# joaotavora/raytracing-one-weekend

Measured on AMD Instinct MI355X. Metric: Msamples/sec (W×H×spp) on cover scene; achieved HBM GB/s vs peak, higher is better.
Workload: dtype f64

## Files before the change

### include/rtow.h

```cpp
#ifndef RTOW_H
#define RTOW_H

#include <stdint.h>

#ifdef __cplusplus
extern "C" {
#endif

#define RTOW_ABI_VERSION 9

#define RTOW_OK 0
#define RTOW_EINVAL (-1)
#define RTOW_ENODEV (-2)
#define RTOW_EHIP (-3)
#define RTOW_ENOSCENE (-4)
#define RTOW_EEMPTY (-5)
#define RTOW_ENOMEM (-6)

#define RTOW_MAT_LAMBERTIAN 0
#define RTOW_MAT_METAL 1
#define RTOW_MAT_DIELECTRIC 2

#define RTOW_PRIM_SPHERE 0
#define RTOW_PRIM_MOVING_SPHERE 1
// ... 101 lines not shown
  int32_t bvh_image_bytes;
  int32_t grid_image_bytes;
  double bvh_build_ms;
  double grid_build_ms;
  double upload_ms;
  int32_t bvh4_nodes;
  int32_t bvh4_image_bytes;
  int32_t ref_tree_nodes;
  int32_t bvh4_node_bytes;
  double ref_tree_stupid_volume;
  double ref_tree_build_ms;
} rtow_build_info_t;
int rtow_build_info(rtow_ctx *ctx, rtow_build_info_t *out);

int rtow_local_rows(const rtow_config_t *cfg);
int rtow_local_row_list(const rtow_config_t *cfg, int32_t *rows_out, int32_t capacity);

int rtow_render_device(rtow_ctx *ctx, const rtow_config_t *cfg, void *d_rgb_sums,
                       void *hip_stream, rtow_stats_t *stats);

int rtow_render_device_rgb8(rtow_ctx *ctx, const rtow_config_t *cfg, void *d_rgb8, void *hip_stream,
                            rtow_stats_t *stats);

int rtow_tonemap_device(rtow_ctx *ctx, const void *d_rgb_sums, int64_t n_values, int32_t spp_effective,
                        void *d_rgb8, void *hip_stream);

int rtow_profile_collect(rtow_ctx *ctx, double *kernel_ms_sum, int32_t *launches);

int rtow_debug_counters(rtow_ctx *ctx, unsigned long long *out48);

int rtow_debug_schedule(rtow_ctx *ctx, const rtow_config_t *cfg, uint32_t *out_pairs, int32_t capacity_pairs);

int rtow_debug_last_spec(rtow_ctx *ctx, uint32_t *out_spec);

int rtow_debug_tile_order(const rtow_scene_t *scene, const rtow_config_t *cfg, uint32_t *table_out, unsigned char *empty_out,
                          int32_t capacity, int32_t *n_empty, int32_t *tile_w_log2, int32_t *tile_h_log2);

int rtow_debug_image(rtow_ctx *ctx, int32_t which, void *out, int64_t capacity, int64_t *size_out);

typedef struct rtow_ray_t {
  double origin[3];
  double time;
  double direction[3];
  double tmax;
} rtow_ray_t;

typedef struct rtow_hit_t {
  double t;
  double point[3];
  double normal[3];
  int32_t prim;
  int32_t kind;
  int32_t material;
  int32_t front_face;
} rtow_hit_t;

int rtow_intersect_device(rtow_ctx *ctx, int32_t precision, int32_t kernel, const void *d_rays, int64_t n_rays,
                          void *d_hits, void *hip_stream, rtow_stats_t *stats);
int rtow_intersect(rtow_ctx *ctx, int32_t precision, int32_t kernel, const rtow_ray_t *rays, int64_t n_rays,
                   rtow_hit_t *hits, rtow_stats_t *stats);

int rtow_occluded_device(rtow_ctx *ctx, int32_t precision, int32_t kernel, const void *d_rays, int64_t n_rays,
                         void *d_occluded , void *hip_stream, rtow_stats_t *stats);
int rtow_occluded(rtow_ctx *ctx, int32_t precision, int32_t kernel, const rtow_ray_t *rays, int64_t n_rays,
                  uint8_t *occluded, rtow_stats_t *stats);

// ... 126 lines not shown
```

### raytracing-one-weekend_amd/csrc/rtow_capi.cpp

```cpp

#include <hip/hip_runtime.h>

#include <cmath>
#include <cstdarg>
#include <cstdio>
#include <cstdlib>
#include <algorithm>
#include <chrono>
#include <cstring>
#include <string>
#include <vector>

#include "../../include/rtow.h"
#include "rtow_bvh.h"
#include "rtow_bvh4.h"
#include "rtow_device.h"
#include "rtow_grid.h"
#include "rtow_reftree.h"

namespace {

thread_local std::string g_err;

int fail(int code, const char *fmt, ...) {
// ... 241 lines not shown
struct Knobs {
  int bvh_leaf = 0;
  double bvh_ct = -1.0;
  bool no_leaf_order = false;
  double grid_cpp = 1.0;
  double grid_large = 4.0;
  int grid_max_tris = 8192;
  unsigned long long partials_cap = 8ull << 30;
  int bvh_block = 0;
  int blocks_per_cu = 0;
  bool no_tiles = false;
  int sky_eighths = 1;
  bool stamps = false;
  bool bvh4_no_aux = false;
  bool no_bvh4 = false;
  int fetch_votes = 0;
  int leaf_votes = 0;
  int walk_cap = -1, walk_max_open = 0;
  bool bvh4_sm = false;
  int sm4_votes[3] = {8, 16, 16};
  int bvh4_stack_k = 0;
  int sched_chunk = 10;
  int sched_chunk_mesh = 16;
  int ploc_radius = -1;
  int device_tree = 2;
  bool stream_scalar = false;
  bool no_spec = false;
  bool no_flat = false;
  bool tile_order = true;
  int empty_levels = 3;
  int tail_bound = 0;
  int radiance_blocks = 0;
  int guides_blocks = 0;
  void read() {
    auto geti = [](const char *n, int d) { const char *e = std::getenv(n); return e ? std::atoi(e) : d; };
    auto getd = [](const char *n, double d) { const char *e = std::getenv(n); return e ? std::atof(e) : d; };
    bvh_leaf = geti("RTOW_BVH_LEAF", 0);
    bvh_ct = getd("RTOW_BVH_CT", -1.0);
    no_leaf_order = std::getenv("RTOW_NO_LEAF_ORDER") != nullptr;
    grid_cpp = getd("RTOW_GRID_CPP", 1.0);
    grid_large = getd("RTOW_GRID_LARGE", 4.0);
    grid_max_tris = geti("RTOW_GRID_MAX_TRIS", 8192);
    if (const char *e = std::getenv("RTOW_PARTIALS_MAX_MB")) partials_cap = (unsigned long long)std::atoll(e) << 20;
    bvh_block = geti("RTOW_BVH_BLOCK", 0);
    if (bvh_block != 256 && bvh_block != 512 && bvh_block != 1024) bvh_block = 0;
    blocks_per_cu = geti("RTOW_BLOCKS_PER_CU", 0);
    if (blocks_per_cu < 1 || blocks_per_cu > 16) blocks_per_cu = 0;
    no_tiles = std::getenv("RTOW_NO_TILES") != nullptr;
    sky_eighths = std::min(std::max(geti("RTOW_SKY_EIGHTHS", 1), 0), 8);
    stamps = std::getenv("RTOW_STAMPS") != nullptr;
    no_bvh4 = std::getenv("RTOW_NO_BVH4") != nullptr;
    bvh4_no_aux = std::getenv("RTOW_BVH4_NO_AUX") != nullptr;
    fetch_votes = std::min(std::max(geti("RTOW_FETCH_VOTES", 0), 0), 64);
    leaf_votes = std::min(std::max(geti("RTOW_LEAF_VOTES", 0), 0), 64);
    bvh4_sm = std::getenv("RTOW_BVH4_SM") != nullptr;
    if (const char *e = std::getenv("RTOW_WALK_CAP")) {
      int a = 0, b = 0;
      if (std::sscanf(e, "%d,%d", &a, &b) == 2 && a > 0 && b > 0) {
        walk_cap = a;
        walk_max_open = std::min(b, 64);
      } else {
        walk_cap = 0;
      }
    }
    if (const char *e = std::getenv("RTOW_SM4_VOTES")) {
      int a = 0, b = 0, d = 0;
      if (std::sscanf(e, "%d,%d,%d", &a, &b, &d) == 3) {
        sm4_votes[0] = std::min(std::max(a, 1), 64);
        sm4_votes[1] = std::min(std::max(b, 1), 64);
        sm4_votes[2] = std::min(std::max(d, 1), 64);
      }
    }
    bvh4_stack_k = std::min(std::max(geti("RTOW_BVH4_STACK_K", 0), 0), 64);
    sched_chunk = std::min(std::max(geti("RTOW_SCHED_CHUNK", 10), 0), 4096);
    sched_chunk_mesh = std::min(std::max(geti("RTOW_SCHED_CHUNK_MESH", 16), 0), 4096);
    tail_bound = std::max(geti("RTOW_TAIL_BOUND", 0), 0);
    radiance_blocks = std::max(geti("RTOW_RADIANCE_BLOCKS", 0), 0);
    guides_blocks = std::max(geti("RTOW_GUIDES_BLOCKS", 0), 0);
    tile_order = geti("RTOW_TILE_ORDER", 1) != 0;
    empty_levels = std::min(std::max(geti("RTOW_EMPTY_LEVELS", 3), 1), 16);
    no_spec = std::getenv("RTOW_NO_SPEC") != nullptr;
    no_flat = std::getenv("RTOW_NO_FLAT") != nullptr;
    stream_scalar = std::getenv("RTOW_STREAM_SCALAR") != nullptr;
    if (const char *e = std::getenv("RTOW_PLOC_RADIUS")) ploc_radius = std::min(std::max(std::atoi(e), 0), 64);
    if (const char *e = std::getenv("RTOW_DEVICE_TREE"))
      device_tree = std::strcmp(e, "radix") == 0 ? 0 : (std::strcmp(e, "ploc") == 0 ? 1 : 2);
    if (ploc_radius >= 0 && !std::getenv("RTOW_DEVICE_TREE")) device_tree = ploc_radius == 0 ? 0 : 1;
  }
};

constexpr unsigned kNeedBvh = 1u, kNeedGrid = 2u, kNeedF32 = 4u, kNeedBvh4 = 8u, kNeedAll = 15u;

struct rtow_ctx {
  int device = 0;
  Knobs knobs;
  int num_cus = 0;
  bool have_scene = false;
  rtow::DevScene ds{};
  rtow::DevCamera cam{};
  int n_prims = 0;
  DevBuf sph, sph_r, mov, tri, tri16, prim_mat, mats, blob, cam_dev, gblob;
  DevBuf blob4;
  bool have_bvh4 = false;
  bool have_tri16 = false;
  int bvh4_depth = 0;
  DevBuf blob32, gblob32, cam32_dev;
  rtow::DevScene ds32{};
  uint32_t gblob_bytes = 0;
  uint32_t grid_fat_stride = 0;
  int32_t grid_ny = 0;
  GridWalkConsts grid_walk{};
// ... 1122 lines not shown
  LaunchShape shape;
  if ((rc = launch_shape(c, kernel, f32, shape))) return rc;
  rtow::DevScene &scene = shape.scene;
  const int block = shape.block;
  const unsigned lds_bytes = shape.lds_bytes;
  const int stack_bound = shape.stack_bound;
  const bool image_kernel = shape.image_kernel;

  if (stats) {
    std::memset(stats, 0, sizeof *stats);
    stats->local_rows = rows;
    stats->kernel_used = kernel;
  }
  if (npix == 0) return RTOW_OK;
  if (spt == 0) {
    if (!accumulate) HIPCHK(hipMemsetAsync(d_rgb_sums, 0, (size_t)npix * 3 * sizeof(double), st));
    if (stats) HIPCHK(hipStreamSynchronize(st));
    return RTOW_OK;
  }

  int &occ = c->occ[strict ? 0 : (f32 ? 2 : 1)][kernel - 1];
  if (kernel == RTOW_KERNEL_BVH4) occ = 0;
  if (occ <= 0) {
    occ = strict ? rtow::trace_occupancy_strict(kernel, block, lds_bytes)
          : f32  ? rtow::trace_occupancy_f32(kernel, block, lds_bytes)
                 : rtow::trace_occupancy_fast(kernel, block, lds_bytes);
    if (occ <= 0) return fail(RTOW_EHIP, "occupancy query failed (kernel %d, %u B of LDS)", kernel, lds_bytes);
    if (occ > 8) occ = 8;
    if (c->knobs.blocks_per_cu) occ = c->knobs.blocks_per_cu;
  }
  long long grid = (long long)c->num_cus * occ;
  const long long need_blocks = (long long)((n_items + block - 1) / block);
  if (grid > need_blocks) grid = need_blocks;
  if (grid < 1) grid = 1;
  const unsigned long long n_lanes = (unsigned long long)grid * block;

  const size_t depth_slots = (size_t)(cfg->max_child_rays > 0 ? cfg->max_child_rays : 1);
  if ((rc = c->partials.ensure((size_t)n_items * 3 * sizeof(double))) ||
      (rc = c->stack.ensure(strict ? depth_slots * (size_t)n_lanes * sizeof(uint32_t) : 4)) ||
      (rc = c->counters.ensure(48 * sizeof(unsigned long long))))
    return rc;
  if (kernel == RTOW_KERNEL_BVH4) {
    const int extra = std::max(stack_bound - (int)scene.b4_stack_k, 0);
    if ((rc = c->spill.ensure(std::max<size_t>((size_t)extra * (size_t)n_lanes * sizeof(uint32_t), 16)))) return rc;
  }

#ifdef RTOW_TAILSTAT
  if (kernel == RTOW_KERNEL_BVH4) return fail(RTOW_EINVAL, "RTOW_TAILSTAT builds do not run the BVH4 kernel");
  if ((rc = c->spill.ensure(std::max<size_t>((size_t)n_lanes, 16)))) return rc;
#endif
  rtow::TraceParams P;
  std::memset(&P, 0, sizeof P);
  P.sc = scene;
  P.cam = (const rtow::DevCamera *)c->cam_dev.p;
  P.cam32 = (const float *)c->cam32_dev.p;
  P.W = cfg->image_width;
  P.H = cfg->image_height;
  P.spt = spt;
  P.nstreams = streams_now;
  P.stream_first = plan.first + lvl_first;
  P.sample_base = (uint32_t)(plan.base + (long long)lvl_first * spt);
  P.spt_last = spt_last;
  {
    const unsigned long long b = 64ull * (4096ull + 8ull * (unsigned long long)(cfg->max_child_rays + 2) *
                                                        (unsigned long long)(std::max(spt, spt_last) + 1));
    P.tail_bound = c->knobs.tail_bound > 0 ? (uint32_t)c->knobs.tail_bound : (uint32_t)std::min<unsigned long long>(b, 0xfffffff0ull);
  }
  P.dropped = (unsigned long long *)c->dropped.p;
  P.inv_wm1 = 1.0 / (double)(cfg->image_width - 1);
  P.inv_hm1 = 1.0 / (double)(cfg->image_height - 1);
  P.max_child_rays = cfg->max_child_rays;
  P.rank = cfg->rank;
  P.nranks = cfg->nranks;
  P.tile_rows = cfg->tile_rows;
  P.local_rows = rows;
  P.seed_lo = (uint32_t)cfg->seed;
  P.seed_hi = (uint32_t)(cfg->seed >> 32);
  P.n_items = (uint32_t)n_items;
  P.n_lanes = (uint32_t)n_lanes;
  P.npix_local = (uint32_t)npix;
  P.div_npix = make_fastdiv((uint32_t)npix);
  P.div_w = make_fastdiv((uint32_t)cfg->image_width);
// ... 26 lines not shown
    }
    P.tile_table = (const uint32_t *)c->tile_table.p;
    P.n_items_first = P.n_items - c->tile_empty * 64u * (uint32_t)streams_now;
    P.empty_batch = 64u * (uint32_t)c->knobs.empty_levels;
  }
  P.partials = (double *)c->partials.p;
  P.stack = (uint32_t *)c->stack.p;
  P.spill = (uint32_t *)c->spill.p;
  P.spec = rtow::kSpecGeneric;
  if (kernel == RTOW_KERNEL_GRID && lds_bytes > 0 && !f32 && !c->knobs.no_spec && scene.n_tri == 0) {
    if (scene.n_mov == 0 && c->grid_fat_stride == 48u) P.spec = rtow::kSpecStaticSpheres;
    if (scene.n_mov > 0 && c->grid_fat_stride == 80u) P.spec = rtow::kSpecMovingSpheres;
    if (P.spec != rtow::kSpecGeneric && c->grid_ny == 1 && !c->knobs.no_flat) P.spec |= rtow::kSpecFlatY;
  }
  P.walk = c->grid_walk;
  P.b4_trips = c->knobs.bvh4_sm ? 0u : 1u;
  {
    const bool b4 = kernel == RTOW_KERNEL_BVH4;
    const bool b4_nodes_resident = b4 && scene.b4_lds_limit >= scene.b4_off_tri;
    int cap = c->knobs.walk_cap, open = c->knobs.walk_max_open;
    if (cap < 0) {
      cap = b4 ? 4 : 3;
      open = b4 ? (b4_nodes_resident ? 24 : 32) : 16;
    }
    if (cap > 0 && !b4) cap = std::max(cap, 3);
    P.walk_cap = cap > 0 ? (uint32_t)cap : 0xffffffffu;
    P.walk_max_open = (uint32_t)open;
    P.leaf_votes = (uint32_t)(c->knobs.leaf_votes > 0 ? c->knobs.leaf_votes : (b4 ? 28 : 16));
  }
  P.fetch_votes = (uint32_t)(c->knobs.fetch_votes > 0 ? c->knobs.fetch_votes : (kernel == RTOW_KERNEL_BVH4 ? 2 : 4));
  P.sm4_restart = (uint32_t)c->knobs.sm4_votes[0];
  P.sm4_scatter = (uint32_t)c->knobs.sm4_votes[1];
  P.sm4_leaf = (uint32_t)c->knobs.sm4_votes[2];
  P.counters = (unsigned long long *)c->counters.p;
  P.t_origin = P.counters + 16;

  if (st != nullptr) HIPCHK(hipStreamWaitEvent(st, c->upload_ev, 0));
  if (stats) HIPCHK(hipEventRecord(c->call_ev[0], st));
  if (!c->counters_init.p) {
    std::vector<unsigned long long> init(48, 0ull);
    init[5] = init[16] = ~0ull;
    if ((rc = c->counters_init.ensure(48 * sizeof(unsigned long long)))) return rc;
    HIPCHK(hipMemcpy(c->counters_init.p, init.data(), 48 * sizeof(unsigned long long), hipMemcpyHostToDevice));
  }
  HIPCHK(hipMemcpyAsync(c->counters.p, c->counters_init.p, 48 * sizeof(unsigned long long), hipMemcpyDeviceToDevice, st));
  const int slot = c->ev_count < kEventRing ? c->ev_count : -1;
  if (slot >= 0) HIPCHK(hipEventRecord(c->ev[slot][0], st));
  int launch_kernel = kernel;
  if (image_kernel && lds_bytes > 0 && c->knobs.stamps) launch_kernel = kernel + 16;
  int lrc = strict ? rtow::launch_trace_strict(P, launch_kernel, (int)grid, block, lds_bytes, st)
            : f32  ? rtow::launch_trace_f32(P, launch_kernel, (int)grid, block, lds_bytes, st)
                   : rtow::launch_trace_fast(P, launch_kernel, (int)grid, block, lds_bytes, st);
#ifdef RTOW_TAILSTAT
  if (const char *path = std::getenv("RTOW_TAILSTAT_OUT")) {
    HIPCHK(hipStreamSynchronize(st));
    std::vector<unsigned long long> ts((size_t)n_lanes / 64 * 8);
    HIPCHK(hipMemcpy(ts.data(), c->spill.p, ts.size() * 8, hipMemcpyDeviceToHost));
    if (FILE *f = std::fopen(path, "wb")) {
      std::fwrite(ts.data(), 8, ts.size(), f);
      std::fclose(f);
    }
  }
#endif
  if (lrc != 0) return fail(RTOW_EHIP, "trace kernel launch failed: %s", hipGetErrorString((hipError_t)lrc));
  c->last_spec = (int64_t)P.spec;
  if (slot >= 0) {
    HIPCHK(hipEventRecord(c->ev[slot][1], st));
    c->ev_count++;
  }
  rtow::ReduceParams R;
  R.partials = P.partials;
  R.out = (double *)d_rgb_sums;
  R.npix3 = (uint32_t)(npix * 3);
  R.nstreams = streams_now;
  R.accumulate = accumulate;
  R.W = (uint32_t)cfg->image_width;
  R.tile_w_log2 = tw;
  R.tile_h_log2 = th;
  R.tiles_per_row = P.div_tpr_n;
  R.rgb8 = nullptr;
  R.spp = 0.0;
  if (c->fuse_rgb8 && lvl_first == 0 && lvl_count == plan.count && !accumulate) {
    R.rgb8 = c->fuse_rgb8;
    R.spp = c->fuse_spp;
    c->fuse_used = true;
  }
  lrc = rtow::launch_reduce(R, st);
  if (lrc != 0) return fail(RTOW_EHIP, "reduce kernel launch failed: %s", hipGetErrorString((hipError_t)lrc));

// ... 553 lines not shown
        frame.half = c->ds.b4_half;
        frame.lds_limit = c->ds.b4_lds_limit;
        bytes = (int64_t)sizeof frame;
      }
      break;
    default: return fail(RTOW_EINVAL, "unknown image %d", which);
  }
  *size_out = bytes;
  if (!out) return RTOW_OK;
  if (capacity < bytes) return fail(RTOW_EINVAL, "buffer too small (%lld < %lld)", (long long)capacity, (long long)bytes);
  if (which == 5) {
    if (bytes) std::memcpy(out, &frame, sizeof frame);
    return RTOW_OK;
  }
  HIPCHK(hipSetDevice(c->device));
  HIPCHK(hipDeviceSynchronize());
  if (bytes) HIPCHK(hipMemcpy(out, src, (size_t)bytes, hipMemcpyDeviceToHost));
  return RTOW_OK;
}

int rtow_debug_counters(rtow_ctx *c, unsigned long long *out48) {
  if (!c || !out48) return fail(RTOW_EINVAL, "NULL argument");
  if (!c->counters.p) return fail(RTOW_ENOSCENE, "no launch yet");
  HIPCHK(hipSetDevice(c->device));
  HIPCHK(hipDeviceSynchronize());
  HIPCHK(hipMemcpy(out48, c->counters.p, 48 * sizeof(unsigned long long), hipMemcpyDeviceToHost));
  return RTOW_OK;
}

int rtow_debug_last_spec(rtow_ctx *c, uint32_t *out_spec) {
  if (!c || !out_spec) return fail(RTOW_EINVAL, "NULL argument");
  if (c->last_spec < 0) return fail(RTOW_ENOSCENE, "no launch yet");
  *out_spec = (uint32_t)c->last_spec;
  return RTOW_OK;
}

int rtow_tonemap_device(rtow_ctx *c, const void *d_rgb_sums, int64_t n_values, int32_t spp_effective,
                        void *d_rgb8, void *hip_stream) {
  if (!c) return fail(RTOW_EINVAL, "ctx is NULL");
  if (!d_rgb_sums || !d_rgb8) return fail(RTOW_EINVAL, "NULL device pointer");
  if (n_values < 0 || n_values > 0xffffffffLL) return fail(RTOW_EINVAL, "n_values out of range");
  if (spp_effective <= 0) return fail(RTOW_EINVAL, "spp_effective must be positive");
  HIPCHK(hipSetDevice(c->device));
  int lrc = rtow::launch_tonemap((const double *)d_rgb_sums, (unsigned char *)d_rgb8, (uint32_t)n_values,
                                 (double)spp_effective, hip_stream);
  if (lrc != 0) return fail(RTOW_EHIP, "tonemap launch failed: %s", hipGetErrorString((hipError_t)lrc));
  return RTOW_OK;
}

int rtow_profile_collect(rtow_ctx *c, double *kernel_ms_sum, int32_t *launches) {
  if (!c) return fail(RTOW_EINVAL, "ctx is NULL");
  HIPCHK(hipSetDevice(c->device));
  double sum = 0.0;
  for (int i = 0; i < c->ev_count; ++i) {
    HIPCHK(hipEventSynchronize(c->ev[i][1]));
    float ms = 0.f;
    HIPCHK(hipEventElapsedTime(&ms, c->ev[i][0], c->ev[i][1]));
    sum += ms;
  }
  if (kernel_ms_sum) *kernel_ms_sum = sum;
  if (launches) *launches = c->ev_count;
  const bool waited = c->ev_count > 0;
  c->ev_count = 0;
  return waited ? check_dropped(c, false) : RTOW_OK;
}

// ... 515 lines not shown
```

### raytracing-one-weekend_amd/csrc/rtow_device.h

```cpp
#pragma once
#include <stdint.h>

#include "rtow_walk_consts.h"

namespace rtow {

struct DevMaterial {
  double att[3];
  double fuzz;
  double ir;
  int32_t kind;
  int32_t pad_;
};

struct DevCamera {
  double origin[3], u[3], v[3];
  double horizontal[3], vertical[3], llc[3];
  double lens_radius, t0, t1;
};

struct DevScene {
  const double *sph;
  const double *sph_r;
  const double *mov;
// ... 51 lines not shown
};
struct alignas(32) FetchHead {
  uint32_t n_items;
  uint32_t n_items_first;
  uint32_t empty_batch;
  int32_t W;
  double *partials;
  unsigned long long *counters;
};
static_assert(sizeof(FetchDecode) == 128 && sizeof(FetchHead) == 32, "aligned runs: one or two wide scalar loads each");

struct TraceParams : FetchDecode, FetchHead {
  DevScene sc;
  const DevCamera *cam;
  const float *cam32;
  int32_t H;
  int32_t stream_first;
  uint32_t tail_bound;
  double inv_wm1, inv_hm1;
  int32_t max_child_rays;
  int32_t local_rows;
  uint32_t seed_lo, seed_hi;
  uint32_t n_lanes;
  FastDiv div_npix, div_w;
  uint32_t n_tile_rows;
  uint32_t *stack;
  uint32_t *spill;
  uint32_t spec;
  uint32_t b4_trips;
  uint32_t fetch_votes;
  uint32_t leaf_votes;
  uint32_t walk_cap, walk_max_open;
  uint32_t sm4_restart, sm4_scatter, sm4_leaf;
  unsigned long long *dropped;
  unsigned long long *t_origin;
  GridWalkConsts walk;
};

constexpr uint32_t kSpecGeneric = 0u, kSpecStaticSpheres = 1u, kSpecMovingSpheres = 2u;
constexpr uint32_t kSpecFlatY = 4u;

struct ReduceParams {
  const double *partials;
  double *out;
  uint32_t npix3;
  int32_t nstreams;
  int32_t accumulate;
  uint32_t W, tile_w_log2, tile_h_log2, tiles_per_row;
  unsigned char *rgb8;
  double spp;
};

int launch_trace_strict(const TraceParams &p, int kernel, int grid, int block, unsigned lds_bytes,
                        void *stream);
int launch_trace_fast(const TraceParams &p, int kernel, int grid, int block, unsigned lds_bytes,
                      void *stream);
int launch_trace_f32(const TraceParams &p, int kernel, int grid, int block, unsigned lds_bytes,
                     void *stream);
int trace_occupancy_strict(int kernel, int block, unsigned lds_bytes);
int trace_occupancy_fast(int kernel, int block, unsigned lds_bytes);
int trace_occupancy_f32(int kernel, int block, unsigned lds_bytes);
int launch_reduce(const ReduceParams &p, void *stream);
int launch_tonemap(const double *sums, unsigned char *rgb8, uint32_t n, double spp, void *stream);
int launch_place_rows(const void *gathered, void *image, uint32_t n_ranks, uint32_t max_rows, uint32_t row_bytes,
                      uint32_t height, uint32_t tile_rows, void *stream);

}
```

### raytracing-one-weekend_amd/csrc/rtow_trace_body.h

```cpp

#include <hip/hip_runtime.h>
#include <stdint.h>
#include <type_traits>

#include "rtow_device.h"

#ifndef RTOW_SUFFIX
#error "define RTOW_SUFFIX"
#endif
#define RTOW_CAT2(a, b) a##b
#define RTOW_CAT(a, b) RTOW_CAT2(a, b)

namespace rtow {
namespace {
#include "rtow_trace_math.h"
#include "rtow_trace_rng.h"
#include "rtow_trace_hit.h"
#include "rtow_trace_stamps.h"
#include "rtow_trace_bvh.h"
#include "rtow_trace_grid.h"
#include "rtow_trace_bvh4.h"
#ifndef RTOW_FAST_MATH
#include "rtow_trace_reftree.h"
#endif
// ... 202 lines not shown
  const unsigned lane = lane_id();
  [[maybe_unused]] const uint32_t lane_g = blockIdx.x * blockDim.x + threadIdx.x;

  Image<LDS> im;
  [[maybe_unused]] Bvh4Reader<LDS> im4;
  stage_scene<KERNEL, LDS>(sc, im, im4);

  bool done = false;
  bool need_sample = true;
  bool pending_hit = false;
  int s_left = 0;
  uint32_t item = 0xffffffffu;
  uint32_t j = 0;
  uint32_t gi = 0;
  V3d acc = {0.0, 0.0, 0.0};
  V3 ro = {0, 0, 0}, rd = {0, 0, 1};
  real rtime = 0;
  int depth = 0;
  [[maybe_unused]] int nb = 0;
#ifdef RTOW_FAST_MATH
  V3 throughput = {1, 1, 1};
#endif
  Rng g = {0, 0, 0};
  uint32_t nseg = 0, nnode = 0, nprim = 0;
  [[maybe_unused]] float t_resume = 0.0f;
  [[maybe_unused]] uint32_t w_cur = 0x1fffffu, w_sa = 0u;
  Closest best;
  best.t = 0;
  best.prim = -1;
  bool helping = false;
  bool holding = false;
  uint32_t partners = 0u;
  int n_out = 0;
  uint32_t tail_left = P.tail_bound;
  asm volatile("" : "+v"(tail_left));
  ItemPool pool;
  const uint32_t n_waves = (gridDim.x * blockDim.x) >> 6;
#ifdef RTOW_TAILSTAT
  unsigned long long ts_start = __builtin_amdgcn_s_memrealtime(), ts_empty = 0ull;
  uint32_t ts_trips = 0u, ts_trips_after = 0u, ts_live = 0u, ts_left = 0u, ts_pool = 0u;
#endif
  Stamps<STAMPS> stamps;
  stamps.start();
  unsigned long long t_empty = 0ull;
  unsigned long long trips_after_empty = 0ull;
  if constexpr (STAMPS) {
    if (lane == 0) atomicMin(P.t_origin, (unsigned long long)__builtin_amdgcn_s_memrealtime());
  }

  for (;;) {
    bool need_item = false;
    if (!done && need_sample && s_left <= 0) {
      if (helping) {
        helping = false;
        holding = true;
        done = true;
      } else if (n_out == 0) {
        need_item = true;
      }
    }
    unsigned long long need_mask = __ballot(need_item);
    if (need_mask != 0ull && (uint32_t)__popcll(need_mask) < P.fetch_votes && __ballot(!done && !need_item) != 0ull) {
      need_mask = 0ull;
      need_item = false;
    }
    if (need_mask != 0ull) {
      const RTOW_CONST TraceParams *kp = (const RTOW_CONST TraceParams *)__builtin_amdgcn_kernarg_segment_ptr();
      asm volatile("" : "+s"(kp));
      const FetchHead fh = load_fetch_head(kp);
      if (need_item && item != 0xffffffffu) {
        double *dst = fh.partials + (size_t)item * 3;
        dst[0] = acc.x;
        dst[1] = acc.y;
        dst[2] = acc.z;
        item = 0xffffffffu;
      }
      const unsigned long long mine = take_items(pool, need_mask, lane, n_waves, fh);
      if (need_item) {
        if (mine >= (unsigned long long)fh.n_items) {
          done = true;
#ifdef RTOW_TAILSTAT
          if (ts_empty == 0ull) ts_empty = 1ull;
#endif
          if constexpr (STAMPS) {
            if (t_empty == 0ull) t_empty = __builtin_amdgcn_s_memrealtime();
          }
        } else {
          const ItemPos ip = decode_item(kp, fh, (uint32_t)mine);
          item = ip.item;
          j = ip.j;
          gi = ip.gi;
          g.pixel = gi * (uint32_t)fh.W + j;
          g.sample = ip.sample0;
          s_left = ip.count;
          acc = {0.0, 0.0, 0.0};
        }
      }
    }
#ifdef RTOW_TAILSTAT
    {
      const bool first = __ballot(ts_empty == 1ull) != 0ull && __ballot(ts_empty > 1ull) == 0ull;
      if (first) {
        const unsigned long long now = __builtin_amdgcn_s_memrealtime();
        ts_live = (uint32_t)__popcll(__ballot(!done));
        uint32_t sl = (!done && s_left > 0) ? (uint32_t)s_left : 0u;
        for (int off = 32; off >= 1; off >>= 1) sl += __shfl_xor(sl, off);
        ts_left = sl;
        ts_pool = pool.end - pool.next;
        ts_empty = now < 2ull ? 2ull : now;
      } else if (__ballot(ts_empty > 1ull) != 0ull) {
        ts_empty = (unsigned long long)__shfl((long long)ts_empty, __ffsll((long long)__ballot(ts_empty > 1ull)) - 1);
      }
      ++ts_trips;
      if (__ballot(ts_empty > 1ull) != 0ull) ++ts_trips_after;
    }
#endif
    if (__ballot(done) != 0ull) {
#ifdef RTOW_DONATE_R2
      const bool ready = !done && need_sample && s_left <= 0 && n_out > 0;
      if (__ballot(ready) != 0ull) {
        const uint32_t h = partners & 63u;
        const uint32_t src = ready ? h : lane;
        const uint32_t partner_holds = lane_read(src, (uint32_t)holding);
        const bool take = ready && partner_holds != 0u;
        const V3d c = {lane_read(src, acc.x), lane_read(src, acc.y), lane_read(src, acc.z)};
        const uint32_t ow = holding ? partners : lane;
        const bool o_take = lane_read(ow, (uint32_t)take) != 0u;
        const uint32_t o_h = lane_read(ow, h);
        if (take) {
          acc = acc + c;
          partners >>= 6;
          --n_out;
        }
        if (holding && o_take && o_h == lane) holding = false;
      }
      const bool can_give = !done && !helping && s_left >= 2 && n_out < 5;
#else
      unsigned long long rm = __ballot(!done && need_sample && s_left <= 0 && n_out > 0);
      while (rm != 0ull) {
        const int o = __ffsll((long long)rm) - 1;
        rm &= rm - 1ull;
        const uint32_t want_sample = (uint32_t)__builtin_amdgcn_readlane((int)g.sample, o);
        const uint32_t want_pixel = (uint32_t)__builtin_amdgcn_readlane((int)g.pixel, o);
        const unsigned long long held =
            __ballot(holding && partners == (uint32_t)o && g.sample == want_sample + 1u && g.pixel == want_pixel);
        if (held != 0ull) {
          const int h = __ffsll((long long)held) - 1;
          const V3d c = {wave_bcast_f64(acc.x, h), wave_bcast_f64(acc.y, h), wave_bcast_f64(acc.z, h)};
          if ((int)lane == o) {
            acc = acc + c;
            ++g.sample;
            --n_out;
          }
          if ((int)lane == h) holding = false;
          if (__builtin_amdgcn_readlane(n_out, o) > 0) rm |= 1ull << o;
        }
      }
      const bool can_give = !done && !helping && s_left >= 2;
#endif
      const bool can_help = done && !holding;
      const unsigned long long gm = __ballot(can_give), hm = __ballot(can_help);
      if (gm != 0ull && hm != 0ull) {
        const uint32_t ng = (uint32_t)__popcll(gm), nh = (uint32_t)__popcll(hm);
        const uint32_t cnt = ng < nh ? ng : nh;
        const uint32_t grank = lanes_below(gm), hrank = lanes_below(hm);
        const uint32_t giver_k = (uint32_t)__builtin_amdgcn_ds_permute(
            (int)((can_give ? grank : ng + (lane - grank)) << 2), (int)lane);
        const bool gives = can_give && grank < cnt;
        const bool helps = can_help && hrank < cnt;
        const uint32_t my_giver = lane_read(helps ? hrank : lane, giver_k);
#ifdef RTOW_DONATE_R2
        const uint32_t helper_k = (uint32_t)__builtin_amdgcn_ds_permute(
            (int)((can_help ? hrank : nh + (lane - hrank)) << 2), (int)lane);
        const uint32_t my_helper = lane_read(gives ? grank : lane, helper_k);
#endif
        const uint32_t gsrc = helps ? my_giver : lane;
        const uint32_t o_j = lane_read(gsrc, j), o_gi = lane_read(gsrc, gi);
        const uint32_t o_pixel = lane_read(gsrc, g.pixel), o_sample = lane_read(gsrc, g.sample);
        const uint32_t o_left = lane_read(gsrc, (uint32_t)s_left);
        if (gives) {
          s_left -= 1;
#ifdef RTOW_DONATE_R2
          partners = (partners << 6) | my_helper;
#endif
          ++n_out;
        }
        if (helps) {
          j = o_j;
          gi = o_gi;
          g.pixel = o_pixel;
          g.sample = o_sample + o_left - 1u;
          s_left = 1;
          need_sample = true;
          acc = {0.0, 0.0, 0.0};
          helping = true;
          done = false;
          partners = my_giver;
        }
      }
      if (tail_left == 0u) {
        if (!done || holding) {
          const RTOW_CONST TraceParams *kpt = (const RTOW_CONST TraceParams *)__builtin_amdgcn_kernarg_segment_ptr();
          atomicAdd(&P.counters[47], 1ull);
          atomicAdd(kpt->dropped, 1ull);
        }
        done = true;
        helping = false;
        holding = false;
        n_out = 0;
      } else {
        --tail_left;
      }
    }
    if (__ballot(!done || holding) == 0ull) break;
    stamps.mark(RG_FETCH);

    const bool live = !done && !(need_sample && s_left <= 0);

    const bool do_regen = live && need_sample;
    const bool do_scat = live && pending_hit;
    V3 normal = anyv3();
    bool front = true;
    int mi = 0, kind = 0;
    real m_fuzz = anyv(real(0)), m_ir = anyv(real(0));
#ifdef RTOW_FAST_MATH
    V3 m_att = anyv3();
#endif
    if (do_scat) {
      ro = ro + rd * best.t;
      const int pid = best.prim;
      if constexpr (KERNEL == 4) {
        const uint32_t r = sc.b4_off_tri + 96u * (uint32_t)pid;
        const vd2 q4 = im4.t2(r + 64u), q5 = im4.t2(r + 80u);
// ... 299 lines not shown
      atomicMax(&P.counters[6], tend - P.t_origin[0]);
      atomicAdd(&P.counters[7], t_empty - P.t_origin[0]);
      {
        const unsigned long long after = tend - t_empty;
        unsigned bin = (unsigned)(after / 20000ull);
        bin = bin > 5u ? 5u : bin;
        atomicAdd(&P.counters[17 + bin], 1ull);
        atomicMax(&P.counters[40], trips_after_empty);
        if (bin >= 2u) {
          atomicAdd(&P.counters[41], trips_after_empty);
          atomicAdd(&P.counters[42], after);
          atomicAdd(&P.counters[43], 1ull);
        }
      }
      for (int r = 0; r < RG_COUNT; ++r) atomicAdd(&P.counters[8 + r], stamps.t[r]);
      for (int r = 0; r < RG_COUNT; ++r) atomicAdd(&P.counters[29 + r], stamps.tt[r]);
      atomicAdd(&P.counters[37], trips_after_empty);
      atomicAdd(&P.counters[38], tend - t_empty);
      for (int r = 0; r < RG_COUNT; ++r) atomicAdd(&P.counters[23 + r], stamps.lt[r]);
      atomicAdd(&P.counters[34], stamps.step_lanes);
      atomicAdd(&P.counters[44], stamps.blocks);
      atomicAdd(&P.counters[36], stamps.block_lanes);
      atomicAdd(&P.counters[35], stamps.leaf_lanes);
      atomicAdd(&P.counters[45], stamps.iters_cam);
      atomicAdd(&P.counters[46], stamps.phases_cam);
      atomicAdd(&P.counters[13], stamps.iters);
      atomicAdd(&P.counters[14], stamps.trips);
      atomicAdd(&P.counters[15], stamps.phases);
    }
  }

#ifdef RTOW_TAILSTAT
  if (lane == 0 && P.spill != nullptr) {
    unsigned long long *ts = (unsigned long long *)P.spill + (size_t)((blockIdx.x * blockDim.x + threadIdx.x) >> 6) * 8;
    ts[0] = ts_start;
    ts[1] = ts_empty;
    ts[2] = __builtin_amdgcn_s_memrealtime();
    ts[3] = ts_trips;
    ts[4] = ts_trips_after;
    ts[5] = ts_live;
    ts[6] = ts_left;
    ts[7] = ts_pool;
  }
#endif
  unsigned long long t0 = nseg, t1 = nprim, t2 = nnode;
#pragma unroll
  for (int off = 32; off >= 1; off >>= 1) {
    t0 += __shfl_down(t0, off);
    t1 += __shfl_down(t1, off);
    t2 += __shfl_down(t2, off);
  }
  if (lane == 0) {
    atomicAdd(&P.counters[1], t0);
    if (KERNEL >= 2) {
      atomicAdd(&P.counters[2], t1);
      atomicAdd(&P.counters[3], t2);
    }
  }
}

#include "rtow_trace_sm4.h"

}

#include "rtow_kernel_launch.h"

template <int K, bool L, bool S, int SPEC = 0>
static KernelVariant<TraceParams> trace_kernel(unsigned lds_bytes) {
  return kernel_variant<RTOW_CAT(rtow_trace_, RTOW_SUFFIX)<K, L, S, SPEC>, TraceParams>(lds_bytes);
}
template <bool L, bool S>
static KernelVariant<TraceParams> trace4_kernel(unsigned lds_bytes) {
  return kernel_variant<RTOW_CAT(rtow_trace4_, RTOW_SUFFIX)<L, S>, TraceParams>(lds_bytes);
}

static KernelVariant<TraceParams> trace_variant(int kernel, unsigned lds_bytes, uint32_t spec, bool b4_full,
                                                bool b4_trips) {
  const bool lds = lds_bytes > 0;
  switch (kernel) {
    case 1: return trace_kernel<1, false, false>(lds_bytes);
    case 2: return lds ? trace_kernel<2, true, false>(lds_bytes) : trace_kernel<2, false, false>(0);
    case 3:
      if (lds && spec == kSpecStaticSpheres) return trace_kernel<3, true, false, 1>(lds_bytes);
      if (lds && spec == kSpecMovingSpheres) return trace_kernel<3, true, false, 2>(lds_bytes);
      if (lds && spec == (kSpecStaticSpheres | kSpecFlatY)) return trace_kernel<3, true, false, 1 | (int)kSpecFlatY>(lds_bytes);
      if (lds && spec == (kSpecMovingSpheres | kSpecFlatY)) return trace_kernel<3, true, false, 2 | (int)kSpecFlatY>(lds_bytes);
// ... 30 lines not shown
```

### raytracing-one-weekend_amd/rtow.py

```python
from __future__ import annotations

import ctypes as C
import os
from pathlib import Path

import numpy as np

PKG_DIR = Path(__file__).resolve().parent
REPO_ROOT = PKG_DIR.parent
LIB_PATH = Path(os.environ.get("RTOW_LIB", PKG_DIR / "librtow.so"))

RTOW_ABI_VERSION = 9
RTOW_OK, RTOW_EINVAL, RTOW_ENODEV, RTOW_EHIP, RTOW_ENOSCENE, RTOW_EEMPTY, RTOW_ENOMEM = 0, -1, -2, -3, -4, -5, -6
MAT_LAMBERTIAN, MAT_METAL, MAT_DIELECTRIC = 0, 1, 2
PRIM_SPHERE, PRIM_MOVING_SPHERE, PRIM_TRIANGLE = 0, 1, 2
F64_STRICT, F64_FAST, F32 = 0, 1, 2
KERNEL_AUTO, KERNEL_BRUTE, KERNEL_BVH, KERNEL_GRID, KERNEL_BVH4, KERNEL_REFTREE = 0, 1, 2, 3, 4, 5
MAX_HITS = 8
SPEC_GENERIC, SPEC_STATIC_SPHERES, SPEC_MOVING_SPHERES, SPEC_FLAT_Y = 0, 1, 2, 4
MODEL_OO, MODEL_VARIANT, MODEL_WORLD = 0, 1, 2
BUILDER_HOST_SAH, BUILDER_DEVICE_LBVH, BUILDER_AUTO = 0, 1, 2

d3 = C.c_double * 3
_pd = C.POINTER(C.c_double)
# ... 121 lines not shown
    q["point"] = p
    q["time"] = time
    q["max_dist"] = max_dist
    q["pad_"] = 0.0
    return q


def make_rays(origins, directions, time=0.0, tmax=float("inf")):
    o = np.asarray(origins, dtype=np.float64).reshape(-1, 3)
    d = np.asarray(directions, dtype=np.float64).reshape(-1, 3)
    r = np.empty(len(o), dtype=RAY_DTYPE)
    r["origin"] = o
    r["direction"] = d
    r["time"] = time
    r["tmax"] = tmax
    return r


EXPORTS = [
    "rtow_abi_version", "rtow_last_error", "rtow_ctx_create", "rtow_ctx_destroy",
    "rtow_scene_upload", "rtow_local_rows", "rtow_local_row_list", "rtow_render_device",
    "rtow_render", "rtow_host_scene_cover", "rtow_host_scene_obj", "rtow_host_scene_free",
    "rtow_host_rng_reset", "rtow_host_ppm", "rtow_host_free", "rtow_tonemap_device",
    "rtow_profile_collect", "rtow_debug_counters", "rtow_render_rgb8",
    "rtow_ctx_set_builder", "rtow_build_info", "rtow_debug_image", "rtow_render_multi",
    "rtow_debug_schedule", "rtow_host_scene_cover_model", "rtow_host_scene_obj_model",
    "rtow_multi_create", "rtow_multi_set_builder", "rtow_multi_upload", "rtow_multi_build_info",
    "rtow_multi_render", "rtow_multi_destroy", "rtow_host_reftree_info",
    "rtow_render_device_rgb8", "rtow_multi_render_rgb8", "rtow_multi_frame_breakdown",
    "rtow_intersect_device", "rtow_intersect", "rtow_occluded_device", "rtow_occluded",
    "rtow_scene_refit", "rtow_refit_info", "rtow_closest_point_device", "rtow_closest_point",
    "rtow_debug_tile_order", "rtow_radiance_device", "rtow_radiance",
    "rtow_camera_rays_device", "rtow_camera_rays", "rtow_camera_ray_count", "rtow_guides_device", "rtow_guides",
    "rtow_debug_last_spec", "rtow_first_hits_device", "rtow_first_hits",
]
MULTI_BREAKDOWN = ("total", "handoff_enqueue", "place_enqueue", "wait_and_copy", "wait_only", "dev_trace", "dev_gather",
                   "dev_place_copy")


class RtowError(RuntimeError):
    pass


_lib = None


def lib():
    global _lib
    if _lib is not None:
        return _lib
    try:
        import torch
    except ImportError:
        pass
    if not LIB_PATH.exists():
        raise RtowError(f"{LIB_PATH} is missing: run `python -c 'import __graft_entry__ as g; g.build()'`"
                        " (there is no CPU fallback)")
    L = C.CDLL(str(LIB_PATH))
    L.rtow_abi_version.restype = C.c_int
    L.rtow_last_error.restype = C.c_char_p
    L.rtow_ctx_create.argtypes = [C.c_int, C.POINTER(C.c_void_p)]
    L.rtow_ctx_destroy.argtypes = [C.c_void_p]
    L.rtow_ctx_destroy.restype = None
    L.rtow_scene_upload.argtypes = [C.c_void_p, C.POINTER(Scene)]
    L.rtow_local_rows.argtypes = [C.POINTER(Config)]
    L.rtow_local_row_list.argtypes = [C.POINTER(Config), _pi, C.c_int32]
    L.rtow_render_device.argtypes = [C.c_void_p, C.POINTER(Config), C.c_void_p, C.c_void_p,
# ... 49 lines not shown
        L.rtow_first_hits_device.argtypes = [C.c_void_p, C.c_int32, C.c_int32, C.c_void_p, C.c_int64, C.c_int32, C.c_void_p,
                                             C.c_void_p, C.c_void_p, C.POINTER(Stats)]
        L.rtow_first_hits.argtypes = [C.c_void_p, C.c_int32, C.c_int32, C.c_void_p, C.c_int64, C.c_int32, C.c_void_p,
                                      C.c_void_p, C.POINTER(Stats)]
    if hasattr(L, "rtow_closest_point"):
        L.rtow_closest_point_device.argtypes = [C.c_void_p, C.c_int32, C.c_int32, C.c_void_p, C.c_int64, C.c_void_p,
                                                C.c_void_p, C.POINTER(Stats)]
        L.rtow_closest_point.argtypes = [C.c_void_p, C.c_int32, C.c_int32, C.c_void_p, C.c_int64, C.c_void_p,
                                         C.POINTER(Stats)]
    if hasattr(L, "rtow_radiance"):
        L.rtow_radiance_device.argtypes = [C.c_void_p, C.c_int32, C.c_int32, C.POINTER(RadianceParams), C.c_void_p, C.c_int64,
                                           C.c_void_p, C.c_void_p, C.c_void_p, C.POINTER(Stats)]
        L.rtow_radiance.argtypes = [C.c_void_p, C.c_int32, C.c_int32, C.POINTER(RadianceParams), C.c_void_p, C.c_int64,
                                    C.c_void_p, C.c_void_p, C.POINTER(Stats)]
    if hasattr(L, "rtow_guides"):
        L.rtow_camera_rays_device.argtypes = [C.c_void_p, C.POINTER(Config), C.c_void_p, C.c_void_p, C.c_void_p]
        L.rtow_camera_rays.argtypes = [C.c_void_p, C.POINTER(Config), C.c_void_p, C.c_void_p]
        L.rtow_camera_ray_count.argtypes = [C.POINTER(Config)]
        L.rtow_camera_ray_count.restype = C.c_int64
        L.rtow_guides_device.argtypes = [C.c_void_p, C.POINTER(Config), C.c_void_p, C.c_void_p, C.POINTER(Stats)]
        L.rtow_guides.argtypes = [C.c_void_p, C.POINTER(Config), C.c_void_p, C.POINTER(Stats)]
    if hasattr(L, "rtow_scene_refit"):
        L.rtow_scene_refit.argtypes = [C.c_void_p, C.POINTER(Scene)]
        L.rtow_refit_info.argtypes = [C.c_void_p, C.POINTER(RefitInfo)]
    L.rtow_profile_collect.argtypes = [C.c_void_p, C.POINTER(C.c_double), C.POINTER(C.c_int32)]
    if hasattr(L, "rtow_debug_schedule"):
        L.rtow_debug_schedule.argtypes = [C.c_void_p, C.POINTER(Config), C.POINTER(C.c_uint32), C.c_int32]
    if hasattr(L, "rtow_debug_tile_order"):
        L.rtow_debug_tile_order.argtypes = [C.POINTER(Scene), C.POINTER(Config), C.POINTER(C.c_uint32),
                                            C.POINTER(C.c_ubyte), C.c_int32, C.POINTER(C.c_int32),
                                            C.POINTER(C.c_int32), C.POINTER(C.c_int32)]
    if hasattr(L, "rtow_debug_last_spec"):
        L.rtow_debug_last_spec.argtypes = [C.c_void_p, C.POINTER(C.c_uint32)]
    ver = L.rtow_abi_version()
    if ver != RTOW_ABI_VERSION and not ("RTOW_LIB" in os.environ and ver >= 4):
        raise RtowError("librtow.so ABI version mismatch")
    _lib = L
    return L


def check(rc: int, what: str = "rtow"):
    if rc != 0:
        msg = lib().rtow_last_error()
        raise RtowError(f"{what} failed ({rc}): {msg.decode() if msg else ''}")


def image_height(width: int, aspect_ratio: float) -> int:
    return int(width / aspect_ratio)


def make_config(width, height, spp, nstreams=1, max_child_rays=50, seed=1, precision=F64_FAST,
                kernel=KERNEL_AUTO, rank=0, nranks=1, tile_rows=8, stream_first=0, stream_count=0,
                accumulate=0) -> Config:
    return Config(width, height, spp, nstreams, max_child_rays, precision, kernel, rank, nranks,
                  tile_rows, seed, stream_first, stream_count, accumulate, 0)


def spp_effective(cfg: Config) -> int:
    return cfg.samples_per_pixel // cfg.nstreams * cfg.nstreams


def local_rows(cfg: Config):
    L = lib()
    n = L.rtow_local_rows(C.byref(cfg))
    if n < 0:
        check(n, "rtow_local_rows")
# ... 73 lines not shown
    def __init__(self, device_id: int = 0):
        self._h = C.c_void_p()
        check(lib().rtow_ctx_create(device_id, C.byref(self._h)), "rtow_ctx_create")
        self.device_id = device_id

    def upload(self, scene):
        s = scene.c if isinstance(scene, HostScene) else scene
        check(lib().rtow_scene_upload(self._h, C.byref(s)), "rtow_scene_upload")

    def refit(self, scene):
        s = scene.c if isinstance(scene, HostScene) else scene
        check(lib().rtow_scene_refit(self._h, C.byref(s)), "rtow_scene_refit")

    def refit_info(self) -> RefitInfo:
        ri = RefitInfo()
        check(lib().rtow_refit_info(self._h, C.byref(ri)), "rtow_refit_info")
        return ri

    def set_builder(self, builder: int):
        check(lib().rtow_ctx_set_builder(self._h, builder), "rtow_ctx_set_builder")

    def debug_image(self, which: int) -> bytes:
        n = C.c_int64()
        check(lib().rtow_debug_image(self._h, which, None, 0, C.byref(n)), "rtow_debug_image")
        buf = (C.c_ubyte * max(n.value, 1))()
        check(lib().rtow_debug_image(self._h, which, buf, n.value, C.byref(n)), "rtow_debug_image")
        return bytes(buf[:n.value])

    def last_spec(self) -> int:
        v = C.c_uint32()
        check(lib().rtow_debug_last_spec(self._h, C.byref(v)), "rtow_debug_last_spec")
        return int(v.value)

    def build_info(self) -> BuildInfo:
        bi = BuildInfo()
        check(lib().rtow_build_info(self._h, C.byref(bi)), "rtow_build_info")
        return bi

    def render_device(self, cfg: Config, d_ptr: int, stream: int = 0, want_stats=False):
        st = Stats() if want_stats else None
        check(lib().rtow_render_device(self._h, C.byref(cfg), C.c_void_p(d_ptr),
                                       C.c_void_p(stream), C.byref(st) if st is not None else None),
              "rtow_render_device")
        return st

    def tonemap_device(self, d_sums: int, n_values: int, spp_eff: int, d_rgb8: int, stream: int = 0):
        check(lib().rtow_tonemap_device(self._h, C.c_void_p(d_sums), n_values, spp_eff,
                                        C.c_void_p(d_rgb8), C.c_void_p(stream)), "rtow_tonemap_device")

    def render(self, scene, cfg: Config, into=None):
        import numpy as np

        s = scene.c if isinstance(scene, HostScene) else scene
        rows = lib().rtow_local_rows(C.byref(cfg))
        if rows < 0:
            check(rows, "rtow_local_rows")
        out = np.zeros((rows, cfg.image_width, 3), dtype=np.float64) if into is None else into
        st = Stats()
        check(lib().rtow_render(self._h, C.byref(s), C.byref(cfg), out.ctypes.data_as(_pd),
                                C.byref(st)), "rtow_render")
        return out, st

    def render_rgb8(self, scene, cfg: Config, want_stats=True):
        import numpy as np

        s = scene.c if isinstance(scene, HostScene) else scene
# ... 236 lines not shown
```

Before: 16960.

## Start intra-wave sample donation early once sky items are reached

```diff
diff --git a/include/rtow.h b/include/rtow.h
--- a/include/rtow.h
+++ b/include/rtow.h
@@ -157,6 +157,8 @@
 int rtow_debug_schedule(rtow_ctx *ctx, const rtow_config_t *cfg, uint32_t *out_pairs, int32_t capacity_pairs);
 
 int rtow_debug_last_spec(rtow_ctx *ctx, uint32_t *out_spec);
+
+int rtow_debug_donations(rtow_ctx *ctx, unsigned long long *out_donated, unsigned long long *out_early);
 
 int rtow_debug_tile_order(const rtow_scene_t *scene, const rtow_config_t *cfg, uint32_t *table_out, unsigned char *empty_out,
                           int32_t capacity, int32_t *n_empty, int32_t *tile_w_log2, int32_t *tile_h_log2);
diff --git a/raytracing-one-weekend_amd/csrc/rtow_capi.cpp b/raytracing-one-weekend_amd/csrc/rtow_capi.cpp
--- a/raytracing-one-weekend_amd/csrc/rtow_capi.cpp
+++ b/raytracing-one-weekend_amd/csrc/rtow_capi.cpp
@@ -297,6 +297,8 @@
   int tail_bound = 0;
   int radiance_blocks = 0;
   int guides_blocks = 0;
+  int trace_blocks = 0;
+  bool early_help = true;
   void read() {
     auto geti = [](const char *n, int d) { const char *e = std::getenv(n); return e ? std::atoi(e) : d; };
     auto getd = [](const char *n, double d) { const char *e = std::getenv(n); return e ? std::atof(e) : d; };
@@ -342,6 +344,8 @@
     tail_bound = std::max(geti("RTOW_TAIL_BOUND", 0), 0);
     radiance_blocks = std::max(geti("RTOW_RADIANCE_BLOCKS", 0), 0);
     guides_blocks = std::max(geti("RTOW_GUIDES_BLOCKS", 0), 0);
+    trace_blocks = std::max(geti("RTOW_TRACE_BLOCKS", 0), 0);
+    early_help = geti("RTOW_EARLY_HELP", 1) != 0;
     tile_order = geti("RTOW_TILE_ORDER", 1) != 0;
     empty_levels = std::min(std::max(geti("RTOW_EMPTY_LEVELS", 3), 1), 16);
     no_spec = std::getenv("RTOW_NO_SPEC") != nullptr;
@@ -1530,6 +1534,7 @@
   long long grid = (long long)c->num_cus * occ;
   const long long need_blocks = (long long)((n_items + block - 1) / block);
   if (grid > need_blocks) grid = need_blocks;
+  if (c->knobs.trace_blocks > 0 && grid > c->knobs.trace_blocks) grid = c->knobs.trace_blocks;
   if (grid < 1) grid = 1;
   const unsigned long long n_lanes = (unsigned long long)grid * block;
 
@@ -1545,7 +1550,7 @@
 
 #ifdef RTOW_TAILSTAT
   if (kernel == RTOW_KERNEL_BVH4) return fail(RTOW_EINVAL, "RTOW_TAILSTAT builds do not run the BVH4 kernel");
-  if ((rc = c->spill.ensure(std::max<size_t>((size_t)n_lanes, 16)))) return rc;
+  if ((rc = c->spill.ensure(std::max<size_t>((size_t)n_lanes * 2, 16)))) return rc;
 #endif
   rtow::TraceParams P;
   std::memset(&P, 0, sizeof P);
@@ -1638,6 +1643,7 @@
   P.sm4_restart = (uint32_t)c->knobs.sm4_votes[0];
   P.sm4_scatter = (uint32_t)c->knobs.sm4_votes[1];
   P.sm4_leaf = (uint32_t)c->knobs.sm4_votes[2];
+  P.early_help = c->knobs.early_help ? 1u : 0u;
   P.counters = (unsigned long long *)c->counters.p;
   P.t_origin = P.counters + 16;
 
@@ -1660,7 +1666,7 @@
 #ifdef RTOW_TAILSTAT
   if (const char *path = std::getenv("RTOW_TAILSTAT_OUT")) {
     HIPCHK(hipStreamSynchronize(st));
-    std::vector<unsigned long long> ts((size_t)n_lanes / 64 * 8);
+    std::vector<unsigned long long> ts((size_t)n_lanes / 64 * 16);
     HIPCHK(hipMemcpy(ts.data(), c->spill.p, ts.size() * 8, hipMemcpyDeviceToHost));
     if (FILE *f = std::fopen(path, "wb")) {
       std::fwrite(ts.data(), 8, ts.size(), f);
@@ -2280,6 +2286,18 @@
   if (!c || !out_spec) return fail(RTOW_EINVAL, "NULL argument");
   if (c->last_spec < 0) return fail(RTOW_ENOSCENE, "no launch yet");
   *out_spec = (uint32_t)c->last_spec;
+  return RTOW_OK;
+}
+
+int rtow_debug_donations(rtow_ctx *c, unsigned long long *out_donated, unsigned long long *out_early) {
+  if (!c || !out_donated || !out_early) return fail(RTOW_EINVAL, "NULL argument");
+  if (!c->counters.p || c->last_spec < 0) return fail(RTOW_ENOSCENE, "no launch yet");
+  HIPCHK(hipSetDevice(c->device));
+  HIPCHK(hipDeviceSynchronize());
+  unsigned long long w[48];
+  HIPCHK(hipMemcpy(w, c->counters.p, sizeof w, hipMemcpyDeviceToHost));
+  *out_donated = w[rtow::kCounterDonated];
+  *out_early = w[rtow::kCounterDonatedEarly];
   return RTOW_OK;
 }
 
diff --git a/raytracing-one-weekend_amd/csrc/rtow_device.h b/raytracing-one-weekend_amd/csrc/rtow_device.h
--- a/raytracing-one-weekend_amd/csrc/rtow_device.h
+++ b/raytracing-one-weekend_amd/csrc/rtow_device.h
@@ -107,6 +107,7 @@
   uint32_t leaf_votes;
   uint32_t walk_cap, walk_max_open;
   uint32_t sm4_restart, sm4_scatter, sm4_leaf;
+  uint32_t early_help;
   unsigned long long *dropped;
   unsigned long long *t_origin;
   GridWalkConsts walk;
@@ -114,6 +115,8 @@
 
 constexpr uint32_t kSpecGeneric = 0u, kSpecStaticSpheres = 1u, kSpecMovingSpheres = 2u;
 constexpr uint32_t kSpecFlatY = 4u;
+
+constexpr int kCounterDonated = 28, kCounterDonatedEarly = 39;
 
 struct ReduceParams {
   const double *partials;
diff --git a/raytracing-one-weekend_amd/csrc/rtow_trace_body.h b/raytracing-one-weekend_amd/csrc/rtow_trace_body.h
--- a/raytracing-one-weekend_amd/csrc/rtow_trace_body.h
+++ b/raytracing-one-weekend_amd/csrc/rtow_trace_body.h
@@ -258,6 +258,10 @@
   bool holding = false;
   uint32_t partners = 0u;
   int n_out = 0;
+  constexpr uint32_t kEndgame = 1u, kExhausted = 2u, kSkyItem = 4u;
+  uint32_t hstate = 0u;
+  uint32_t n_helped = 0u, n_helped_early = 0u;
+  asm volatile("" : "+v"(hstate), "+v"(n_helped), "+v"(n_helped_early));
   uint32_t tail_left = P.tail_bound;
   asm volatile("" : "+v"(tail_left));
   ItemPool pool;
@@ -265,6 +269,12 @@
 #ifdef RTOW_TAILSTAT
   unsigned long long ts_start = __builtin_amdgcn_s_memrealtime(), ts_empty = 0ull;
   uint32_t ts_trips = 0u, ts_trips_after = 0u, ts_live = 0u, ts_left = 0u, ts_pool = 0u;
+  unsigned long long ts_sky = 0ull;
+  uint32_t ts_sky_trip = 0u, ts_sky_lanes = 0u, ts_sky_unstarted = 0u, ts_empty_unstarted = 0u;
+  auto ts_sum = [](uint32_t v) {
+    for (int off = 32; off >= 1; off >>= 1) v += __shfl_xor(v, off);
+    return v;
+  };
 #endif
   Stamps<STAMPS> stamps;
   stamps.start();
@@ -273,6 +283,14 @@
   if constexpr (STAMPS) {
     if (lane == 0) atomicMin(P.t_origin, (unsigned long long)__builtin_amdgcn_s_memrealtime());
   }
+
+  auto can_give_fn = [](bool done, bool helping, int s_left, [[maybe_unused]] int n_out, uint32_t hstate, bool all) {
+#ifdef RTOW_DONATE_R2
+    return !done && !helping && s_left >= 2 && n_out < 5 && (all || (hstate & kSkyItem) == 0u);
+#else
+    return !done && !helping && s_left >= 2 && (all || (hstate & kSkyItem) == 0u);
+#endif
+  };
 
   for (;;) {
     bool need_item = false;
@@ -300,6 +318,18 @@
         dst[1] = acc.y;
         dst[2] = acc.z;
         item = 0xffffffffu;
+      }
+      if (pool.seen > (unsigned long long)fh.n_items_first &&
+          ((uint32_t)__builtin_amdgcn_readfirstlane((int)hstate) & (kEndgame | kExhausted)) == kEndgame) {
+        const unsigned long long gm = __ballot(can_give_fn(done, helping, s_left, n_out, hstate, false));
+        if (gm != 0ull) {
+          const bool pick = need_item && lanes_below(need_mask) < (uint32_t)__popcll(gm);
+          if (pick) {
+            need_item = false;
+            done = true;
+          }
+          need_mask &= ~__ballot(pick);
+        }
       }
       const unsigned long long mine = take_items(pool, need_mask, lane, n_waves, fh);
       if (need_item) {
@@ -322,6 +352,25 @@
           acc = {0.0, 0.0, 0.0};
         }
       }
+      [[maybe_unused]] const bool bought_sky =
+          pool.seen > (unsigned long long)fh.n_items_first && fh.n_items_first < fh.n_items;
+      if (pool.seen > (unsigned long long)fh.n_items_first) {
+        if (need_item) hstate = (hstate & ~kSkyItem) | (mine >= (unsigned long long)fh.n_items_first ? kSkyItem : 0u);
+        const uint32_t phase = (uint32_t)__builtin_amdgcn_readfirstlane((int)hstate) & (kEndgame | kExhausted);
+        if (__ballot(need_item && done) != 0ull)
+          hstate |= kExhausted;
+        else if (phase == 0u && fh.n_items_first < fh.n_items && kp->early_help != 0u)
+          hstate |= kEndgame;
+      }
+#ifdef RTOW_TAILSTAT
+      if (ts_sky == 0ull && bought_sky) {
+        const bool holds = !done && !helping && (hstate & kSkyItem) == 0u && s_left > 0;
+        ts_sky_lanes = (uint32_t)__popcll(__ballot(holds));
+        ts_sky_unstarted = ts_sum(holds ? (uint32_t)s_left - (need_sample ? 0u : 1u) : 0u);
+        ts_sky_trip = ts_trips;
+        ts_sky = __builtin_amdgcn_s_memrealtime();
+      }
+#endif
     }
 #ifdef RTOW_TAILSTAT
     {
@@ -332,6 +381,8 @@
         uint32_t sl = (!done && s_left > 0) ? (uint32_t)s_left : 0u;
         for (int off = 32; off >= 1; off >>= 1) sl += __shfl_xor(sl, off);
         ts_left = sl;
+        ts_empty_unstarted =
+            ts_sum(!done && !helping && (hstate & kSkyItem) == 0u && s_left > 0 ? (uint32_t)s_left - (need_sample ? 0u : 1u) : 0u);
         ts_pool = pool.end - pool.next;
         ts_empty = now < 2ull ? 2ull : now;
       } else if (__ballot(ts_empty > 1ull) != 0ull) {
@@ -360,7 +411,6 @@
         }
         if (holding && o_take && o_h == lane) holding = false;
       }
-      const bool can_give = !done && !helping && s_left >= 2 && n_out < 5;
 #else
       unsigned long long rm = __ballot(!done && need_sample && s_left <= 0 && n_out > 0);
       while (rm != 0ull) {
@@ -382,8 +432,9 @@
           if (__builtin_amdgcn_readlane(n_out, o) > 0) rm |= 1ull << o;
         }
       }
-      const bool can_give = !done && !helping && s_left >= 2;
-#endif
+#endif
+      const bool exhausted = ((uint32_t)__builtin_amdgcn_readfirstlane((int)hstate) & kExhausted) != 0u;
+      const bool can_give = can_give_fn(done, helping, s_left, n_out, hstate, exhausted);
       const bool can_help = done && !holding;
       const unsigned long long gm = __ballot(can_give), hm = __ballot(can_help);
       if (gm != 0ull && hm != 0ull) {
@@ -422,9 +473,17 @@
           helping = true;
           done = false;
           partners = my_giver;
-        }
-      }
-      if (tail_left == 0u) {
+          n_helped += 1u;
+          n_helped_early += exhausted ? 0u : 1u;
+        }
+      }
+      if (!exhausted) {
+        if (done && !holding) {
+          done = false;
+          need_sample = true;
+          s_left = 0;
+        }
+      } else if (tail_left == 0u) {
         if (!done || holding) {
           const RTOW_CONST TraceParams *kpt = (const RTOW_CONST TraceParams *)__builtin_amdgcn_kernarg_segment_ptr();
           atomicAdd(&P.counters[47], 1ull);
@@ -790,7 +849,7 @@
 
 #ifdef RTOW_TAILSTAT
   if (lane == 0 && P.spill != nullptr) {
-    unsigned long long *ts = (unsigned long long *)P.spill + (size_t)((blockIdx.x * blockDim.x + threadIdx.x) >> 6) * 8;
+    unsigned long long *ts = (unsigned long long *)P.spill + (size_t)((blockIdx.x * blockDim.x + threadIdx.x) >> 6) * 16;
     ts[0] = ts_start;
     ts[1] = ts_empty;
     ts[2] = __builtin_amdgcn_s_memrealtime();
@@ -799,17 +858,31 @@
     ts[5] = ts_live;
     ts[6] = ts_left;
     ts[7] = ts_pool;
+    ts[8] = ts_sky;
+    ts[9] = ts_sky_lanes;
+    ts[10] = ts_sky_unstarted;
+    ts[11] = ts_empty_unstarted;
+    ts[12] = ts_sum(n_helped);
+    ts[13] = ts_sum(n_helped_early);
+    ts[14] = ts_sky_trip;
+    ts[15] = 0ull;
   }
 #endif
   unsigned long long t0 = nseg, t1 = nprim, t2 = nnode;
+  unsigned long long t3 = ((unsigned long long)n_helped_early << 32) | n_helped;
 #pragma unroll
   for (int off = 32; off >= 1; off >>= 1) {
     t0 += __shfl_down(t0, off);
     t1 += __shfl_down(t1, off);
     t2 += __shfl_down(t2, off);
+    t3 += __shfl_down(t3, off);
   }
   if (lane == 0) {
     atomicAdd(&P.counters[1], t0);
+    if (t3 != 0ull) {
+      atomicAdd(&P.counters[kCounterDonated], t3 & 0xffffffffull);
+      atomicAdd(&P.counters[kCounterDonatedEarly], t3 >> 32);
+    }
     if (KERNEL >= 2) {
       atomicAdd(&P.counters[2], t1);
       atomicAdd(&P.counters[3], t2);
diff --git a/raytracing-one-weekend_amd/rtow.py b/raytracing-one-weekend_amd/rtow.py
--- a/raytracing-one-weekend_amd/rtow.py
+++ b/raytracing-one-weekend_amd/rtow.py
@@ -177,7 +177,7 @@
     "rtow_scene_refit", "rtow_refit_info", "rtow_closest_point_device", "rtow_closest_point",
     "rtow_debug_tile_order", "rtow_radiance_device", "rtow_radiance",
     "rtow_camera_rays_device", "rtow_camera_rays", "rtow_camera_ray_count", "rtow_guides_device", "rtow_guides",
-    "rtow_debug_last_spec", "rtow_first_hits_device", "rtow_first_hits",
+    "rtow_debug_last_spec", "rtow_first_hits_device", "rtow_first_hits", "rtow_debug_donations",
 ]
 MULTI_BREAKDOWN = ("total", "handoff_enqueue", "place_enqueue", "wait_and_copy", "wait_only", "dev_trace", "dev_gather",
                    "dev_place_copy")
@@ -293,6 +293,8 @@
                                             C.POINTER(C.c_int32), C.POINTER(C.c_int32)]
     if hasattr(L, "rtow_debug_last_spec"):
         L.rtow_debug_last_spec.argtypes = [C.c_void_p, C.POINTER(C.c_uint32)]
+    if hasattr(L, "rtow_debug_donations"):
+        L.rtow_debug_donations.argtypes = [C.c_void_p, C.POINTER(C.c_ulonglong), C.POINTER(C.c_ulonglong)]
     ver = L.rtow_abi_version()
     if ver != RTOW_ABI_VERSION and not ("RTOW_LIB" in os.environ and ver >= 4):
         raise RtowError("librtow.so ABI version mismatch")
@@ -432,6 +434,11 @@
         check(lib().rtow_debug_last_spec(self._h, C.byref(v)), "rtow_debug_last_spec")
         return int(v.value)
 
+    def donations(self):
+        d, e = C.c_ulonglong(), C.c_ulonglong()
+        check(lib().rtow_debug_donations(self._h, C.byref(d), C.byref(e)), "rtow_debug_donations")
+        return int(d.value), int(e.value)
+
     def build_info(self) -> BuildInfo:
         bi = BuildInfo()
         check(lib().rtow_build_info(self._h, C.byref(bi)), "rtow_build_info")
```

Result: no change. 16950 (-0.1%).
